# Nicholasli1995/EgoNet

Measured on AMD Instinct MI355X. Metric: crops/sec (256x256, heatmap+decode+lift), higher is better.
Workload: dtype f32; 1 GPU; configs[1]: batch=64 256x256 crops/GPU, HRNet-W48 heatmap head forward + soft decode + affine + FC lifter + pose solve; global_batch=64, weights=synthetic (egonet_amd.synth, seeded per key), parallelism=replicas x1, crops sharded by rank, no collective, ranks=1, backend=none, launch_lanes=1

## Files before the change

egonet_amd/_lib.py:

```python
import ctypes as C
import os

_HERE = os.path.dirname(os.path.abspath(__file__))
LIB_PATH = os.environ.get('EGONET_AMD_LIB') or os.path.join(_HERE, 'csrc', 'libegonet_hip.so')
HEADER_PATH = os.path.join(os.path.dirname(_HERE), 'include', 'egonet_hip.h')

ACT_NONE, ACT_RELU, ACT_SIGMOID, ACT_LEAKY = 0, 1, 2, 3


class Ref(C.Structure):
    _fields_ = [('slot', C.c_int32), ('off', C.c_int64)]


NULL_REF = Ref(-1, 0)

_p = C.c_void_p
_i = C.c_int
_d = C.c_double

SIGNATURES = {
    'egn_version': (_i, []),
    'egn_strerror': (C.c_char_p, [_i]),
    'egn_conv2d_f32': (_i, [_p] * 6 + [_i] * 14 + [_p]),
    'egn_conv_plan_query': (_i, [_i] * 13 + [C.POINTER(_i)]),
# ... 86 lines not shown
    'egn_optim_item_floats': (_i, []),
    'egn_optim_grouped_step_f32': (_i, [_i, _p, _p, _p, _p, _p, C.c_long, _p, _p, _i, _p, _p, C.c_long, _p, _p, _p]),
    'egn_grad_norm_ws_bytes': (C.c_long, []),
    'egn_grad_norm_clip_f32': (_i, [_p, C.c_long, C.c_float, _p, _p, _p]),
    'egn_program_create': (_p, [_i]),
    'egn_program_destroy': (None, [_p]),
    'egn_program_bind': (_i, [_p, _i, _p]),
    'egn_program_num_ops': (_i, [_p]),
    'egn_program_add_conv2d': (_i, [_p] + [Ref] * 6 + [_i] * 14),
    'egn_program_add_fuse': (_i, [_p, Ref, _i, _i, _i, _i, _i, _i, C.POINTER(Ref), C.POINTER(_i), _i]),
    'egn_program_add_nchw_to_nhwc': (_i, [_p, Ref, Ref, _i, _i, _i, _i, _i]),
    'egn_program_add_nhwc_to_nchw': (_i, [_p, Ref, Ref, _i, _i, _i, _i, _i]),
    'egn_program_add_pixel_shuffle': (_i, [_p, Ref, Ref, _i, _i, _i, _i, _i, _i]),
    'egn_program_add_pw_pair': (_i, [_p] + [Ref] * 8 + [_i, _i]),
    'egn_program_add_conv2d_pair': (_i, [_p] + ([Ref] * 6 + [_i] * 6) * 2 + [_i]),
    'egn_conv_pair_plan_query': (_i, [_i] * 13 + [C.POINTER(_i)]),
    'egn_conv3x3_h_applies': (_i, [_i] * 9),
    'egn_conv3x3_h_wpack_bytes': (C.c_long, [_i, _i]),
    'egn_conv3x3_h_f32': (_i, [_p] * 6 + [_i] * 6 + [_p]),
    'egn_program_add_conv3x3_h': (_i, [_p] + [Ref] * 6 + [_i] * 6),
    'egn_conv3x3s2_h_applies': (_i, [_i] * 8),
    'egn_conv3x3s2_h_f32': (_i, [_p] * 5 + [_i] * 6 + [_p]),
    'egn_program_add_conv3x3s2_h': (_i, [_p] + [Ref] * 5 + [_i] * 6),
    'egn_conv3x3_hx_applies': (_i, [_i] * 10),
    'egn_conv3x3_hx_wpack_bytes': (C.c_long, [_i, _i]),
    'egn_conv3x3_hx_f32': (_i, [_p] * 6 + [_i] * 7 + [_p]),
    'egn_program_add_conv3x3_hx': (_i, [_p] + [Ref] * 6 + [_i] * 7),
    'egn_pw_pair_f32': (_i, [_p] * 8 + [_i, _i, _p]),
    'egn_program_add_ramps': (_i, [_p, Ref, _i, _i, _i, _i, _i]),
    'egn_program_add_decode': (_i, [_p, Ref, _i, _i, _i, _i, _i, Ref, Ref, Ref]),
    'egn_program_fork': (_i, [_p]),
    'egn_program_join': (_i, [_p]),
    'egn_program_set_lane': (_i, [_p, _i]),
    'egn_program_tag': (_i, [_p, C.c_char_p, _d, _d]),
    'egn_program_run': (_i, [_p, _p]),
    'egn_program_run_timed': (_i, [_p, _p, C.POINTER(C.c_float), _i]),
    'egn_program_capture': (_i, [_p, _p]),
    'egn_program_replay': (_i, [_p, _p]),
    'egn_program_ticket_ops': (_i, [_p]),
    'egn_program_poke_ticket': (_i, [_p, _i, _i, C.c_uint]),
    'egn_gemm_supported': (_i, [_i] * 7),
    'egn_gemm_ws_bytes': (C.c_long, [_i] * 4),
    'egn_gemm_f32': (_i, [_i, _p, _p, _p, _p] + [_i] * 7 + [_p, C.c_long, _p]),
    'egn_gemm_stats_rows': (C.c_long, [_i]),
    'egn_gemm_ex_f32': (_i, [_i, _p, _p, _p, _p, _p, _p, C.c_long] + [_i] * 7 + [_p, C.c_long, _p]),
    'egn_launch_count': (C.c_long, []),
    'egn_direct_conv_count': (C.c_long, []),
    'egn_lifter_pairs_ws_bytes': (C.c_long, [_i, _i]),
    'egn_lifter_pairs_f64': (_i, [_p, _p, _i, _p, _i, _p, _i, _d, _d, _i, _i, _p, C.c_long, _p, _p, _p, _p]),
    'egn_col_mean_std_ws_bytes': (C.c_long, [_i]),
    'egn_col_mean_std_f32': (_i, [_p, C.c_long, _i, _p, C.c_long, _p, _p, _p]),
    'egn_normalize_rows_f32': (_i, [_p, C.c_long, _i, _p, _p, _p]),
    'egn_gather_rows_f32': (_i, [_p, C.c_long, _i, _p, _i, _p, _p]),
    'egn_pose2d_annot_ws_bytes': (C.c_long, [_i]),
    'egn_pose2d_annot_f64': (_i, [_p, _p, _p, _i, _p, _i, _d, _d, _i, _d, _i, _d, _p, C.c_long] + [_p] * 9),
    'egn_lifter_metrics_ws_bytes': (C.c_long, [C.c_long]),
    'egn_lifter_metrics_reset': (_i, [_p, _i, _p]),
    'egn_lifter_metrics_update_f32': (_i, [_p, _p, C.c_long, _i, _i, _p, _p, _i, _p, C.c_long, _p, _p, _p]),
    'egn_kpt_metrics_ws_bytes': (C.c_long, [_i, _i]),
    'egn_kpt_metrics_reset': (_i, [_p, _p]),
    'egn_kpt_metrics_update_f32': (_i, [_p, _p, _i, _i, _i, _i, _i, _p, _p, _p, _p, _i, _d, _d, _p, C.c_long, _p, _p, _p,
                                        _p, _p]),
    'egn_angle_metrics_ws_bytes': (C.c_long, [C.c_long]),
    'egn_angle_metrics_reset': (_i, [_p, _p]),
    'egn_angle_metrics_update_f32': (_i, [_p, C.c_long, _i, _p, _p, C.c_long, _p, _p]),
    'egn_pnp_refine_f64': (_i, [_p] * 5 + [_i, _i, _d] + [_p] * 6 + [_p]),
# ... 55 lines not shown
```

egonet_amd/csrc/program.hip:

```cpp
#include <stdlib.h>
#include <string.h>

#include <string>
#include <atomic>
#include <vector>

#include "egn_internal.h"

extern "C" int egn_conv_config_kind(int cfg);

extern "C" int egn_version(void) { return (1 << 16) | 0; }

extern "C" const char* egn_strerror(int code) {
  if (code == 0) return "ok";
  if (code == EGN_E_BADARG) return "egonet_hip: bad argument / unsupported shape";
  if (code == EGN_E_LDS) return "egonet_hip: tile does not fit in LDS";
  if (code == EGN_E_STATE) return "egonet_hip: program in wrong state";
  if (code > 0) return hipGetErrorString((hipError_t)code);
  return "egonet_hip: unknown error";
}

static int fill_conv_args(ConvArgs& a, const float* x, const float* wpack, const float* scale,
                          const float* shift, const float* res, float* y, int N, int H, int W, int Cin,
                          int cs_in, int Cout, int cs_out, int KH, int KW, int stride, int pad, int act,
// ... 102 lines not shown
  int rc = fill_conv_args(a, nullptr, nullptr, nullptr, nullptr, nullptr, nullptr, N, H, W, Cin, cs_in, Cout,
                          cs_out, KH, KW, stride, pad, 0, out_nchw);
  if (rc) return rc;
  size_t lds;
  rc = egn_conv_plan(a, cfg, lds);
  if (rc) return rc;
  int tm, tn;
  egn_conv_config_info(cfg, &tm, &tn);
  const ConvConfig* cf = egn_conv_config(cfg);
  out[0] = cfg; out[1] = cf->wm; out[2] = cf->wn; out[3] = cf->mt; out[4] = cf->nt;
  out[5] = a.TH; out[6] = a.TW; out[7] = a.TNB; out[8] = a.tps; out[9] = (int)lds;
  out[10] = a.tiles_x * a.tiles_y * ((a.N + a.TNB - 1) / a.TNB);
  out[11] = (a.CoutP + tn - 1) / tn;
  if (egn_conv_config_kind(cfg) == 1 && egn_wino_cot(Cout)) out[11] = Cout / egn_wino_cot(Cout);
  return 0;
}

enum OpKind { OP_CONV = 1, OP_FUSE = 2, OP_NCHW2NHWC = 3, OP_NHWC2NCHW = 4, OP_RAMPS = 5, OP_DECODE = 6,
              OP_FORK = 7, OP_JOIN = 8, OP_PIXSHUF = 9, OP_PWPAIR = 10, OP_CONVPAIR = 11, OP_CONVH = 12, OP_CONVH2 = 13,
              OP_CONVHX = 14 };
constexpr int kMaxLanes = 4;

struct Op {
  int kind;
  int lane = 0;
  ConvArgs conv;
  ConvArgs conv2;
  ConvHArgs convh;
  int cfg;
  egn_ref r[12];
  int i[12];
  std::string tag;
  double flops, bytes;
};

struct egn_program {
  std::vector<void*> slots;
  std::vector<Op> ops;
  std::vector<void*> owned;
  hipGraph_t graph = nullptr;
  hipGraphExec_t exec = nullptr;
  int cur_lane = 0;
  hipStream_t side[kMaxLanes] = {nullptr, nullptr, nullptr, nullptr};
  hipEvent_t ev_fork = nullptr;
  hipEvent_t ev_join[kMaxLanes] = {nullptr, nullptr, nullptr, nullptr};
  hipEvent_t ev_done = nullptr;
  hipStream_t last_stream = nullptr;
  bool ran = false;
  std::vector<unsigned*> tickets;
  std::vector<size_t> ticket_words;
  unsigned** err_ptrs = nullptr;
  unsigned* err_dev = nullptr;
  unsigned* err_host = nullptr;
  hipStream_t init_stream = nullptr;
};

__global__ void egn_ticket_errors_kernel(unsigned** bufs, int n, unsigned* any) {
  unsigned e = 0;
  for (int k = threadIdx.x; k < n; k += 64)
    if (bufs[k][0]) { e = 1u; bufs[k][0] = 0u; }
  if (e) *any = 1u;
}

static int issue_ticket_check(egn_program* p, hipStream_t s) {
  if (p->tickets.empty()) return 0;
  if (!p->err_ptrs) {
    EGN_CHECK_HIP(hipMalloc(&p->err_ptrs, p->tickets.size() * sizeof(unsigned*)));
    EGN_CHECK_HIP(hipMalloc(&p->err_dev, sizeof(unsigned)));
    EGN_CHECK_HIP(hipHostMalloc(&p->err_host, sizeof(unsigned), hipHostMallocDefault));
    *p->err_host = 0u;
    EGN_CHECK_HIP(hipMemcpy(p->err_ptrs, p->tickets.data(), p->tickets.size() * sizeof(unsigned*), hipMemcpyHostToDevice));
    EGN_CHECK_HIP(hipMemset(p->err_dev, 0, sizeof(unsigned)));
  }
  hipLaunchKernelGGL(egn_ticket_errors_kernel, dim3(1), dim3(64), 0, s, p->err_ptrs, (int)p->tickets.size(), p->err_dev);
  EGN_CHECK_HIP(hipGetLastError());
  EGN_CHECK_HIP(hipMemcpyAsync(p->err_host, p->err_dev, sizeof(unsigned), hipMemcpyDeviceToHost, s));
  return 0;
}
// ... 25 lines not shown
static inline void* resolve(const egn_program* p, const egn_ref& r) {
  if (r.slot < 0) return nullptr;
  return (char*)p->slots[r.slot] + r.off;
}
static inline bool ref_ok(const egn_program* p, const egn_ref& r) {
  return r.slot < (int)p->slots.size();
}

extern "C" egn_program* egn_program_create(int nslots) {
  if (nslots < 1 || nslots > 64) return nullptr;
  egn_program* p = new egn_program();
  p->slots.assign(nslots, nullptr);
  return p;
}

static void wait_for_last_run(egn_program* p) {
  if (p->ev_done && p->ran) hipEventSynchronize(p->ev_done);
}

extern "C" void egn_program_destroy(egn_program* p) {
  if (!p) return;
  wait_for_last_run(p);
  if (p->exec) hipGraphExecDestroy(p->exec);
  if (p->graph) hipGraphDestroy(p->graph);
  for (void* d : p->owned) hipFree(d);
  if (p->err_ptrs) hipFree(p->err_ptrs);
  if (p->err_dev) hipFree(p->err_dev);
  if (p->err_host) hipHostFree(p->err_host);
  if (p->init_stream) hipStreamDestroy(p->init_stream);
  for (int k = 1; k < kMaxLanes; ++k) {
    if (p->side[k]) hipStreamDestroy(p->side[k]);
    if (p->ev_join[k]) hipEventDestroy(p->ev_join[k]);
  }
  if (p->ev_fork) hipEventDestroy(p->ev_fork);
  if (p->ev_done) hipEventDestroy(p->ev_done);
  delete p;
}

extern "C" int egn_program_bind(egn_program* p, int slot, void* base) {
  if (!p || slot < 0 || slot >= (int)p->slots.size()) return EGN_E_BADARG;
  if (p->slots[slot] != base && p->exec) {
    wait_for_last_run(p);
    hipGraphExecDestroy(p->exec); p->exec = nullptr;
    hipGraphDestroy(p->graph); p->graph = nullptr;
  }
  p->slots[slot] = base;
  return 0;
}

extern "C" int egn_program_num_ops(const egn_program* p) { return p ? (int)p->ops.size() : 0; }

extern "C" int egn_program_add_conv2d(egn_program* p, egn_ref x, egn_ref wpack, egn_ref scale, egn_ref shift,
                                      egn_ref res, egn_ref y, int N, int H, int W, int Cin, int cs_in,
                                      int Cout, int cs_out, int KH, int KW, int stride, int pad, int act,
                                      int out_nchw, int cfg) {
  if (!p) return EGN_E_BADARG;
  Op op;
  op.kind = OP_CONV;
  op.flops = op.bytes = 0;
  int rc = fill_conv_args(op.conv, nullptr, nullptr, nullptr, nullptr, nullptr, nullptr, N, H, W, Cin, cs_in,
                          Cout, cs_out, KH, KW, stride, pad, act, out_nchw);
  if (rc) return rc;
  if (out_nchw && res.slot >= 0) return EGN_E_BADARG;
  size_t lds;
  rc = egn_conv_plan(op.conv, cfg, lds);
  if (rc) return rc;
// ... 208 lines not shown
  op.kind = OP_PWPAIR;
  op.r[0] = h; op.r[1] = res; op.r[2] = w3; op.r[3] = shift3; op.r[4] = w1; op.r[5] = shift1; op.r[6] = out; op.r[7] = hn;
  for (int k = 0; k < 8; ++k)
    if (!ref_ok(p, op.r[k])) return EGN_E_BADARG;
  op.i[0] = M; op.i[1] = relu1;
  op.flops = 2.0 * M * 64.0 * 256.0 * (w1.slot >= 0 ? 2.0 : 1.0);
  op.bytes = 4.0 * M * (64.0 + 256.0 * (res.slot >= 0 ? 2.0 : 1.0) + (w1.slot >= 0 ? 64.0 : 0.0));
  op.lane = p->cur_lane;
  p->ops.push_back(op);
  return 0;
}

extern "C" int egn_program_fork(egn_program* p) {
  if (!p) return EGN_E_BADARG;
  Op op;
  op.kind = OP_FORK;
  op.flops = op.bytes = 0;
  p->cur_lane = 0;
  p->ops.push_back(op);
  return 0;
}
extern "C" int egn_program_join(egn_program* p) {
  if (!p) return EGN_E_BADARG;
  Op op;
  op.kind = OP_JOIN;
  op.flops = op.bytes = 0;
  p->cur_lane = 0;
  p->ops.push_back(op);
  return 0;
}
extern "C" int egn_program_set_lane(egn_program* p, int lane) {
  if (!p || lane < 0 || lane >= kMaxLanes) return EGN_E_BADARG;
  p->cur_lane = lane;
  return 0;
}

extern "C" int egn_program_tag(egn_program* p, const char* tag, double flops, double bytes) {
  if (!p || p->ops.empty()) return EGN_E_STATE;
  Op& op = p->ops.back();
  op.tag = tag ? tag : "";
  if (flops > 0) op.flops = flops;
  op.bytes = bytes;
  return 0;
}

extern "C" int egn_program_op_info(const egn_program* p, int i, int* kind, double* flops, double* bytes,
                                   char* tag, int tag_len) {
  if (!p || i < 0 || i >= (int)p->ops.size()) return EGN_E_BADARG;
  const Op& op = p->ops[i];
  if (kind) *kind = op.kind;
  if (flops) *flops = op.flops;
  if (bytes) *bytes = op.bytes;
  if (tag && tag_len > 0) {
    strncpy(tag, op.tag.c_str(), tag_len - 1);
    tag[tag_len - 1] = 0;
  }
  return 0;
}

static std::atomic<long> g_launches{0};
static thread_local bool t_recording = false;
extern "C" long egn_launch_count(void) { return g_launches.load(std::memory_order_relaxed); }
void egn_count_launches(long n) { g_launches.fetch_add(n, std::memory_order_relaxed); }

static int launch_op(egn_program* p, Op& op, hipStream_t s) {
  if (!t_recording) g_launches.fetch_add(1, std::memory_order_relaxed);
// ... 35 lines not shown
      int shifts[4];
      for (int k = 0; k < op.i[5]; ++k) {
        terms[k] = (const float*)resolve(p, op.r[1 + k]);
        shifts[k] = op.i[6 + k];
      }
      return egn_fuse_sum_relu_f32((float*)resolve(p, op.r[0]), op.i[0], op.i[1], op.i[2], op.i[3], op.i[4],
                                   op.i[5], terms, shifts, op.i[10], s);
    }
    case OP_NCHW2NHWC:
      return egn_nchw_to_nhwc_f32((const float*)resolve(p, op.r[0]), (float*)resolve(p, op.r[1]), op.i[0],
                                  op.i[1], op.i[2], op.i[3], op.i[4], s);
    case OP_NHWC2NCHW:
      return egn_nhwc_to_nchw_f32((const float*)resolve(p, op.r[0]), (float*)resolve(p, op.r[1]), op.i[0],
                                  op.i[1], op.i[2], op.i[3], op.i[4], s);
    case OP_PIXSHUF:
      return egn_pixel_shuffle_nhwc_to_nchw_f32((const float*)resolve(p, op.r[0]), (float*)resolve(p, op.r[1]),
                                                op.i[0], op.i[1], op.i[2], op.i[3], op.i[4], op.i[5], s);
    case OP_RAMPS:
      return egn_fill_coord_ramps_f32((float*)resolve(p, op.r[0]), op.i[0], op.i[1], op.i[2], op.i[3],
                                      op.i[4], s);
    case OP_PWPAIR:
      return egn_pw_pair_f32((const float*)resolve(p, op.r[0]), (const float*)resolve(p, op.r[1]),
                             (const float*)resolve(p, op.r[2]), (const float*)resolve(p, op.r[3]),
                             (const float*)resolve(p, op.r[4]), (const float*)resolve(p, op.r[5]),
                             (float*)resolve(p, op.r[6]), (float*)resolve(p, op.r[7]), op.i[0], op.i[1], s);
    case OP_DECODE:
      return egn_decode_heatmaps_f32((const float*)resolve(p, op.r[0]), op.i[0], op.i[1], op.i[2], op.i[3],
                                     op.i[4], (float*)resolve(p, op.r[1]), (float*)resolve(p, op.r[2]),
                                     (int32_t*)resolve(p, op.r[3]), s);
  }
  return EGN_E_BADARG;
}

static int ensure_lanes(egn_program* p) {
  if (p->ev_fork) return 0;
  EGN_CHECK_HIP(hipEventCreateWithFlags(&p->ev_fork, hipEventDisableTiming));
  for (int k = 1; k < kMaxLanes; ++k) {
    EGN_CHECK_HIP(hipStreamCreateWithFlags(&p->side[k], hipStreamNonBlocking));
    EGN_CHECK_HIP(hipEventCreateWithFlags(&p->ev_join[k], hipEventDisableTiming));
  }
  return 0;
}

extern "C" int egn_program_run(egn_program* p, void* stream) {
  if (!p) return EGN_E_BADARG;
  hipStream_t main = (hipStream_t)stream;
  bool used[kMaxLanes] = {false, false, false, false};
  bool capturing = false;
  int rc_o = order_behind_last_run(p, main, &capturing);
  if (rc_o) return rc_o;
  if (!capturing) {
    rc_o = consume_ticket_error(p, main);
    if (rc_o) return rc_o;
  }
  for (Op& op : p->ops) {
    if (op.kind == OP_FORK) {
      int rc = ensure_lanes(p);
      if (rc) return rc;
      EGN_CHECK_HIP(hipEventRecord(p->ev_fork, main));
      for (int k = 1; k < kMaxLanes; ++k) used[k] = false;
      continue;
    }
    if (op.kind == OP_JOIN) {
      for (int k = 1; k < kMaxLanes; ++k)
        if (used[k]) {
          EGN_CHECK_HIP(hipEventRecord(p->ev_join[k], p->side[k]));
          EGN_CHECK_HIP(hipStreamWaitEvent(main, p->ev_join[k], 0));
          used[k] = false;
        }
      continue;
    }
    hipStream_t s = main;
    if (op.lane > 0 && p->ev_fork) {
      if (!used[op.lane]) {
        EGN_CHECK_HIP(hipStreamWaitEvent(p->side[op.lane], p->ev_fork, 0));
        used[op.lane] = true;
      }
      s = p->side[op.lane];
    }
    int rc = launch_op(p, op, s);
    if (rc) return rc;
  }
  if (!capturing || p->err_ptrs) {
    int rc = issue_ticket_check(p, main);
    if (rc) return rc;
  }
  return mark_run_issued(p, main, capturing);
}

extern "C" int egn_program_run_timed(egn_program* p, void* stream, float* ms, int n_ms) {
  if (!p || !ms || n_ms < (int)p->ops.size()) return EGN_E_BADARG;
  hipStream_t s = (hipStream_t)stream;
  const size_t n = p->ops.size();
  std::vector<hipEvent_t> ev(n + 1);
  for (auto& e : ev) EGN_CHECK_HIP(hipEventCreate(&e));
  bool capturing = false;
  int rc = order_behind_last_run(p, s, &capturing);
  if (!rc && capturing) rc = EGN_E_STATE;
  if (!rc) rc = consume_ticket_error(p, s);
  if (rc) { for (auto& e : ev) hipEventDestroy(e); return rc; }
  EGN_CHECK_HIP(hipEventRecord(ev[0], s));
  for (size_t i = 0; i < n && !rc; ++i) {
    if (p->ops[i].kind != OP_FORK && p->ops[i].kind != OP_JOIN) rc = launch_op(p, p->ops[i], s);
    if (!rc) rc = (int)hipEventRecord(ev[i + 1], s);
  }
  if (!rc) rc = issue_ticket_check(p, s);
  if (!rc) rc = mark_run_issued(p, s, false);
  if (!rc) rc = (int)hipStreamSynchronize(s);
  if (!rc)
    for (size_t i = 0; i < n; ++i) {
      float t = 0.f;
      hipEventElapsedTime(&t, ev[i], ev[i + 1]);
      ms[i] = t;
    }
  for (auto& e : ev) hipEventDestroy(e);
  return rc;
}

extern "C" int egn_program_ticket_ops(const egn_program* p) { return p ? (int)p->tickets.size() : 0; }
extern "C" int egn_program_poke_ticket(egn_program* p, int op, int word, unsigned value) {
  if (!p || op < 0 || op >= (int)p->tickets.size() || word < 0 || (size_t)word >= p->ticket_words[op]) return EGN_E_BADARG;
  wait_for_last_run(p);
  EGN_CHECK_HIP(hipMemcpy(p->tickets[op] + word, &value, sizeof(unsigned), hipMemcpyHostToDevice));
  return 0;
}

extern "C" int egn_program_capture(egn_program* p, void* stream) {
  if (!p) return EGN_E_BADARG;
  hipStream_t s = (hipStream_t)stream;
  if (p->exec) { wait_for_last_run(p); hipGraphExecDestroy(p->exec); p->exec = nullptr; }
  if (p->graph) { hipGraphDestroy(p->graph); p->graph = nullptr; }
  for (const Op& op : p->ops)
    if (op.kind == OP_FORK) {
      int rc0 = ensure_lanes(p);
      if (rc0) return rc0;
      break;
    }
  EGN_CHECK_HIP(hipStreamBeginCapture(s, hipStreamCaptureModeThreadLocal));
  t_recording = true;
  int rc = egn_program_run(p, stream);
  t_recording = false;
  hipGraph_t g = nullptr;
  hipError_t e = hipStreamEndCapture(s, &g);
  if (rc) { if (g) hipGraphDestroy(g); return rc; }
  if (e != hipSuccess) return (int)e;
  p->graph = g;
  EGN_CHECK_HIP(hipGraphInstantiate(&p->exec, p->graph, nullptr, nullptr, 0));
  return 0;
}

extern "C" int egn_program_replay(egn_program* p, void* stream) {
  if (!p || !p->exec) return EGN_E_STATE;
  long nk = 0;
  for (const Op& op : p->ops) nk += (op.kind != OP_FORK && op.kind != OP_JOIN);
  g_launches.fetch_add(nk, std::memory_order_relaxed);
  bool capturing = false;
  int rc = order_behind_last_run(p, (hipStream_t)stream, &capturing);
  if (rc) return rc;
  if (!capturing) {
    rc = consume_ticket_error(p, (hipStream_t)stream);
    if (rc) return rc;
  }
  EGN_CHECK_HIP(hipGraphLaunch(p->exec, (hipStream_t)stream));
  return mark_run_issued(p, (hipStream_t)stream, capturing);
}
```

egonet_amd/engine.py:

```python
import ctypes as C

import numpy as np
import torch
import torch.nn as nn

from . import _lib, tuner
from ._lib import Ref, NULL_REF, ACT_NONE, ACT_RELU, ACT_SIGMOID, ACT_LEAKY
from .filters import (CK, H_CK, H_KS, _round_up, pack_conv_weight, wino_cot, pack_wino_weight,
                      pack_wino43_weight, pack_wino4_weight, pack_conv_weight_f16, unpack_conv_weight_f16,
                      pack_conv_weight_f16x, unpack_conv_weight_f16x, pack_for_kind)

ACT_RES_AFTER = 0x10
BN_EPS_DEFAULT = 1e-5
SLOT_ARENA, SLOT_WEIGHTS, SLOT_USER0 = 0, 1, 2
PRECISIONS = ('f32', 'f16', 'f16s2')
F16S2_FP32_CLASSES = ((48, 48),)
ALL_PRECISIONS = PRECISIONS + ('f16x',)
_PRECISION_TEXT = "'f32', 'f16', 'f16s2' or 'f16x'"
F16X_FP32_CLASSES = ()


def _h_applies(n, h, w, cin, cs_in, cout, cs_out, has_res, act):
    return bool(_lib.lib().egn_conv3x3_h_applies(n, h, w, cin, cs_in, cout, cs_out, int(has_res), act))


def f16_eligible(conv, n, h, w):
    if not isinstance(conv, nn.Conv2d):
        return False
    if (tuple(conv.kernel_size), tuple(conv.stride), tuple(conv.padding), tuple(conv.dilation), conv.groups) != \
            ((3, 3), (1, 1), (1, 1), (1, 1), 1) or conv.bias is not None or conv.padding_mode != 'zeros':
        return False
    cin, cout = conv.in_channels, conv.out_channels
    return _h_applies(n, h, w, cin, cin, cout, cout, False, ACT_RELU)
# ... 89 lines not shown

def fold_pw(weight, bn):
    cout, cin = weight.shape[:2]
    scale, shift = fold_scale_shift(cout, None, bn)
    w = weight.detach().double().cpu().reshape(cout, cin) * scale[:cout].double()[:, None]
    return w.float().reshape(-1).contiguous(), shift[:cout].clone()


class Buf(object):
    __slots__ = ('n', 'h', 'w', 'c', 'cs', 'slot', 'off', 'nbytes', 'first', 'last', 'uses', 'name')

    def __init__(self, n, h, w, c, cs=None, slot=SLOT_ARENA, nbytes=None, name=''):
        self.n, self.h, self.w, self.c = n, h, w, c
        self.cs = _round_up(c, 4) if cs is None else cs
        self.slot = slot
        self.off = 0
        self.nbytes = nbytes if nbytes is not None else n * h * w * self.cs * 4
        self.first = self.last = -1
        self.uses = []
        self.name = name

    def ref(self):
        return Ref(self.slot, self.off)


class _Recorder(object):
    def __init__(self):
        self.ops = []
        self.blobs = []
        self.blob_off = 0
        self.bufs = []
        self.region = 0
        self.cur_lane = 0
        self.f16 = False
        self.f16s2 = False
        self.f16x = False

    def _push(self, kind, op):
        op['region'], op['lane'] = self.region, self.cur_lane
        self.ops.append((kind, op))

    def fork(self):
        self.region += 1
        self.cur_lane = 0
        self._push('fork', {})

    def lane(self, k):
        self.cur_lane = k % 4

    def join(self):
        self.cur_lane = 0
        self._push('join', {})
        self.region += 1

    def happens_before(self, u, d):
        (ru, lu), (rd, ld) = [(self.ops[i][1]['region'], self.ops[i][1]['lane']) for i in (u, d)]
        return ru < rd or (ru == rd and lu == ld and u < d)

    def new(self, n, h, w, c, name=''):
        b = Buf(n, h, w, c, name=name)
        self.bufs.append(b)
        return b

    def weight(self, t):
        off = self.blob_off
        self.blobs.append(t)
        self.blob_off += _round_up(t.numel() * 4, 256)
        return Ref(SLOT_WEIGHTS, off)

    def _touch(self, *bufs):
        i = len(self.ops)
        for b in bufs:
            if b is None:
                continue
            if b.first < 0:
                b.first = i
            b.last = i
            b.uses.append(i)

    def conv(self, x, weight, bias=None, bn=None, act=ACT_NONE, res=None, stride=1, pad=0,
             dst=None, out_nchw=False, cout_cs=None, tag=''):
        cout, cin, kh, kw = weight.shape
        assert cin == x.c, (cin, x.c, tag)
        ho = (x.h + 2 * pad - kh) // stride + 1
        wo = (x.w + 2 * pad - kw) // stride + 1
        dst_given = dst is not None
        if dst is None:
            dst = self.new(x.n, ho, wo, cout, name=tag)
            if cout_cs is not None:
                dst.cs = cout_cs
# ... 301 lines not shown
            x = op['x']
            _lib.check(L.egn_program_add_nhwc_to_nchw(h, x.ref(), op['y'], x.n, op['c'], x.h, x.w, x.cs))
            nbytes = 8.0 * x.n * x.h * x.w * op['c']
            klass = 'nhwc2nchw %d@%dx%d' % (op['c'], x.h, x.w)
        elif kind == 'pixshuf':
            x = op['x']
            _lib.check(L.egn_program_add_pixel_shuffle(h, x.ref(), op['y'], x.n, op['c'], x.h, x.w, x.cs, op['up']))
            nbytes = 8.0 * x.n * x.h * x.w * op['c'] * op['up'] ** 2
            klass = 'pixel_shuffle%d %d@%dx%d' % (op['up'], op['c'], x.h, x.w)
        elif kind == 'pwpair':
            hb, rb, ob, nb = op['h'], op['res'], op['out'], op['hn']
            none = NULL_REF
            _lib.check(L.egn_program_add_pw_pair(h, hb.ref(), rb.ref() if rb is not None else none, op['w3'], op['shift3'],
                                                 op['w1'] if nb is not None else none,
                                                 op['shift1'] if nb is not None else none, ob.ref(),
                                                 nb.ref() if nb is not None else none, op['m'], op['relu1']))
            flops = 2.0 * op['m'] * 64 * 256 * (2 if nb is not None else 1)
            nbytes = 4.0 * op['m'] * (64 + 256 * (2 if rb is not None else 1) + (64 if nb is not None else 0))
            klass = 'pwpair%d%d 64->256%s@%dx%d' % (int(rb is not None), op['relu1'], '->64' if nb is not None else '',
                                                    hb.h, hb.w)
        elif kind == 'ramps':
            y = op['y']
            _lib.check(L.egn_program_add_ramps(h, y.ref(), y.n, y.h, y.w, y.cs, op['c0']))
            nbytes = 8.0 * y.n * y.h * y.w
            klass = 'ramps'
        elif kind == 'decode':
            _lib.check(L.egn_program_add_decode(h, op['hm'], op['n'], op['k'], op['h'], op['w'],
                                                op['mode'], op['xy'], op['mx'], op['idx']))
            nbytes = 4.0 * op['n'] * op['k'] * op['h'] * op['w']
            klass = 'decode%d %dx%d' % (op['mode'], op['h'], op['w'])
        else:
            raise ValueError(kind)
        L.egn_program_tag(h, (op.get('tag') or klass).encode(), flops, nbytes)
        self.meta.append(dict(kind=kind, klass=klass, tag=op.get('tag', ''), flops=flops, bytes=nbytes,
                              cfg=op.get('cfg', 0) if kind == 'conv' else 0))

    def bind(self, slot, tensor):
        _lib.check(self.lib.egn_program_bind(self.handle, slot, _lib.ptr(tensor)))

    def run(self):
        _lib.check(self.lib.egn_program_run(self.handle, _lib.current_stream(self.device)), 'program_run')

    def run_timed(self):
        n = self.lib.egn_program_num_ops(self.handle)
        ms = (C.c_float * n)()
        _lib.check(self.lib.egn_program_run_timed(self.handle, _lib.current_stream(self.device), ms, n))
        return np.array(ms[:], dtype=np.float64)

    def capture(self):
        _lib.check(self.lib.egn_program_capture(self.handle, _lib.current_stream(self.device)))

    def replay(self):
        _lib.check(self.lib.egn_program_replay(self.handle, _lib.current_stream(self.device)))

    def __del__(self):
        try:
            if getattr(self, 'handle', None):
                self.lib.egn_program_destroy(self.handle)
                self.handle = None
        except Exception:
            pass


class _Stamp(object):

    def __init__(self, model):
# ... 10 lines not shown
            addr ^= t.data_ptr()
        return (ver, addr, len(self.tensors), getattr(self.model, '_egn_generation', 0),
                self.tensors[0].device if self.tensors else None)

    def changed(self):
        now = self._now()
        if now != self.last:
            self.tensors = None
            self.last = self._now()
            return True
        return False


def invalidate(model):
    model._egn_generation = getattr(model, '_egn_generation', 0) + 1
    model._engine = None


def _act_of(seq):
    return ACT_RELU if any(isinstance(m, nn.ReLU) for m in seq) else ACT_NONE


class HRNetEngine(object):

    def __init__(self, model):
        import os
        self.model = model
        self.programs = {}
        self._stamp = _Stamp(model)
        self.lanes = os.environ.get('EGONET_AMD_LANES', '1') != '0'
        self.graph_max_n = int(os.environ.get('EGONET_AMD_GRAPH_MAX_N', '0'))
        self.fuse_layer1 = os.environ.get('EGONET_AMD_PW_FUSE', '1') != '0'
        self.chain_regions = os.environ.get('EGONET_AMD_CHAIN', '1') != '0'
        self.last_f16_ops = []

    @property
    def precision(self):
        prec = getattr(self.model, 'precision', 'f32')
        if prec not in ALL_PRECISIONS:
            raise ValueError("precision must be %s, got %r" % (_PRECISION_TEXT, prec))
        return prec

    def _block(self, r, x, blk, tag):
        y = x
        for i in range(1, blk.depth + 1):
            conv = getattr(blk, 'conv%d' % i)
            bn = getattr(blk, 'bn%d' % i)
            k = conv.kernel_size[0]
            if i < blk.depth:
                y = r.conv(y, conv.weight, None, bn, ACT_RELU, None, conv.stride[0], conv.padding[0],
                           tag='%s.conv%d' % (tag, i))
            else:
                if blk.downsample is None:
                    res = x
                else:
                    pc, pb = blk.downsample[0], blk.downsample[1]
                    res = r.conv(x, pc.weight, None, pb, ACT_NONE, None, pc.stride[0], 0,
                                 tag=tag + '.downsample')
                y = r.conv(y, conv.weight, None, bn, ACT_RELU, res, conv.stride[0], conv.padding[0],
                           tag='%s.conv%d' % (tag, i))
        return y

    def _layer1(self, r, x, blocks):
        def plain():
            t = x
            for k, blk in enumerate(blocks):
# ... 46 lines not shown
            lowered = [any(r.takes_f16(x, conv.weight, conv.bias, ACT_RELU, None, conv.stride[0], conv.padding[0]) or
                           (getattr(r, 'f16x', False) and
                            r.takes_f16x(x, conv.weight, conv.bias, ACT_RELU, None, conv.stride[0], conv.padding[0]))
                           for blk in b for conv in (blk.conv1, blk.conv2) if getattr(blk, 'depth', 0) == 2)
                       for b, x in zip(mod.branches, xs)]

        def plain(branch, x):
            for blk in branch:
                if getattr(blk, 'depth', 0) != 2 or blk.downsample is not None:
                    return False
                for conv in (blk.conv1, blk.conv2):
                    if tuple(conv.weight.shape) != (x.c, x.c, 3, 3) or conv.stride[0] != 1 or conv.padding[0] != 1 \
                            or conv.bias is not None:
                        return False
            return x.cs == x.c and len(branch) > 0

        def key(x, has_res):
            return (x.n, x.h, x.w, x.c, x.c, x.c, x.c, 3, 3, 1, 1, has_res, False)
        nb = mod.num_branches
        for ia in reversed(range(nb)):
            for ib in reversed(range(nb)):
                if ia == ib or len(mod.branches[ia]) != len(mod.branches[ib]) or lowered[ia] or lowered[ib]:
                    continue
                if not (plain(mod.branches[ia], xs[ia]) and plain(mod.branches[ib], xs[ib])):
                    continue
                if all(tuner.pair_usable(key(xs[ia], res), key(xs[ib], res)) for res in (False, True)):
                    return ia, ib
        return None

    def _module(self, r, xs, mod, tag, region_open=False, keep_open=False, nxt=None):
        xs = list(xs)
        pair = self._pair_branches(r, xs, mod)
        lanes = self.lanes and mod.num_branches > 1
        if lanes and not region_open:
            r.fork()
        for b, branch in enumerate(mod.branches):
            if pair is not None and b == max(pair):
                continue
            if lanes:
                r.lane(b)
            if pair is not None and b == min(pair):
                ia, ib = pair
                for k, (ba, bb) in enumerate(zip(mod.branches[ia], mod.branches[ib])):
                    q = '%s.branches.%d+%d.%d' % (tag, ia, ib, k)
                    ha, hb = r.conv_pair(xs[ia], ba.conv1, ba.bn1, ACT_RELU, None,
                                         xs[ib], bb.conv1, bb.bn1, ACT_RELU, None, tag=q + '.conv1')
                    xs[ia], xs[ib] = r.conv_pair(ha, ba.conv2, ba.bn2, ACT_RELU, xs[ia],
                                                 hb, bb.conv2, bb.bn2, ACT_RELU, xs[ib], tag=q + '.conv2')
                continue
            for k, blk in enumerate(branch):
                xs[b] = self._block(r, xs[b], blk, '%s.branches.%d.%d' % (tag, b, k))
        if lanes:
            r.join()
        if mod.fuse_layers is None:
            return xs, False
        outs = []
        stay = lanes and keep_open and self.chain_regions and len(mod.fuse_layers) == mod.num_branches
        pair_next = self._pair_branches(r, xs, nxt) if stay else None
        if lanes:
            r.fork()
        for i, row in enumerate(mod.fuse_layers):
            if lanes:
                r.lane(min(pair_next) if pair_next is not None and i in pair_next else i)
            terms = []
            for j in range(mod.num_branches):
                q = '%s.fuse_layers.%d.%d' % (tag, i, j)
                if row[j] is None:
                    terms.append((xs[j], 0))
                elif j > i:
                    conv, bn = row[j][0], row[j][1]
                    t = r.conv(xs[j], conv.weight, None, bn, ACT_NONE, None, 1, 0, tag=q)
                    terms.append((t, j - i))
                else:
                    terms.append((self._unit_chain(r, xs[j], row[j], q), 0))
            outs.append(r.fuse(terms, True, tag='%s.fuse%d' % (tag, i)))
        if lanes and not stay:
            r.join()
        return outs, stay

    def _record(self, n, cin, h, w, decode_mode, r=None):
        m = self.model
        own = r is None
        if own:
            r = _Recorder()
            r.f16 = self.precision in ('f16', 'f16s2', 'f16x')
            r.f16s2 = self.precision in ('f16s2', 'f16x')
            r.f16x = self.precision == 'f16x'
        x = r.nchw_to_nhwc(Ref(SLOT_USER0, 0), n, cin, h, w, tag='input')
        t = r.conv(x, m.conv1.weight, None, m.bn1, ACT_RELU, None, 2, 1, tag='conv1')
        t = r.conv(t, m.conv2.weight, None, m.bn2, ACT_RELU, None, 2, 1, tag='conv2')
        t = self._layer1(r, t, m.layer1)
        ys = [t]
        for idx in (1, 2, 3):
            trans = getattr(m, 'transition%d' % idx)
            xs = []
            for i, tr in enumerate(trans):
                if tr is None:
                    xs.append(ys[i])
                elif isinstance(tr[0], nn.Conv2d):
                    xs.append(r.conv(ys[-1], tr[0].weight, None, tr[1], ACT_RELU, None, 1, 1,
                                     tag='transition%d.%d' % (idx, i)))
                else:
                    xs.append(self._unit_chain(r, ys[-1], tr, 'transition%d.%d' % (idx, i)))
            stage = getattr(m, 'stage%d' % (idx + 1))
            open_ = False
            for k, mod in enumerate(stage):
                nxt = stage[k + 1] if k + 1 < len(stage) else None
# ... 274 lines not shown
```

egonet_amd/tuner.py:

```python
import atexit
import ctypes as C
import functools
import json
import os

import torch

from . import _lib, filters

_HERE = os.path.dirname(os.path.abspath(__file__))
TABLE_PATH = os.path.join(_HERE, 'tuned', 'gfx950.json')
_table = None
_tuned_here = {}

DIRECT = frozenset((filters.DIRECT,))
ALL_KINDS = frozenset((filters.DIRECT, filters.WINO2, filters.WINO43, filters.WINO4))
TAPE_WINO, TAPE_F43 = frozenset((filters.DIRECT, filters.WINO2)), frozenset((filters.DIRECT, filters.WINO2, filters.WINO4))
F43_KINDS = frozenset((filters.WINO43, filters.WINO4))


def _load():
    global _table
    if _table is None:
        _table = {}
# ... 114 lines not shown
    fit = {int(k): v for k, v in entry.get('ms', {}).items() if ok(int(k))}
    return min(fit, key=fit.get) if fit else 0


def choose(device, key, kinds=DIRECT, ticket_cap=None, inplace_res=False):
    key, kinds = tuple(key), frozenset(kinds)
    mode = os.environ.get('EGONET_AMD_WINO', '')
    if os.environ.get('EGONET_AMD_F43', '1') == '0' or mode in ('0', '1'):
        kinds = kinds - F43_KINDS
    if mode == '0':
        kinds = DIRECT
    elif mode in ('1', '43', '43b', '43w'):
        first = {'43': (70, 80), '43b': (80, 70), '43w': (86, 80, 70)}.get(mode, ())
        ids = list(range(_lib.lib().egn_conv_num_configs(), 0, -1))
        for kind in sorted(kinds - DIRECT, reverse=True):
            for cfg in (list(first) if kind == filters.WINO4 else []) + ids:
                if kind_of(cfg) == kind and usable(key, cfg, kinds, ticket_cap, inplace_res):
                    return cfg
    name = shape_key(*key)
    only = os.environ.get('EGONET_AMD_F43_MATCH', '')
    if only and only not in name:
        kinds = kinds - F43_KINDS
    entry = _load().get(name)
    if entry is None:
        if os.environ.get('EGONET_AMD_AUTOTUNE', '1') == '0':
            return 0
        if name not in _tuned_here:
            cfg, times = tune(device, key)
            _tuned_here[name] = {'cfg': cfg, 'ms': {str(k): round(v, 5) for k, v in times.items()}}
        entry = _tuned_here[name]
    return _pick(entry, key, kinds, ticket_cap, inplace_res)


PAIRS_PATH = os.path.join(_HERE, 'tuned', 'gfx950_pairs.json')
PAIR_CFGS = (86, 82)
PAIR_DEFAULT = '0'
_pairs = None


def _load_pairs():
    global _pairs
    if _pairs is None:
        _pairs = {}
        try:
            with open(PAIRS_PATH) as f:
                _pairs = {k: v for k, v in json.load(f).items() if not k.startswith('_')}
        except (OSError, ValueError):
            _pairs = {}
    return _pairs


def pair_key(key_a, key_b):
    return shape_key(*key_a) + '+' + shape_key(*key_b)


def pair_plans(key_a, key_b, cus=256):
    if any(tuple(k[7:11]) != (3, 3, 1, 1) or k[3] != k[4] or k[5] != k[6] or k[12] for k in (key_a, key_b)):
        return None
    out = (C.c_int * 2)()
    rc = _lib.lib().egn_conv_pair_plan_query(*key_a[:4], key_a[5], *key_b[:4], key_b[5], cus, 0, 0, out)
    return (out[0], out[1]) if rc == 0 else None


def pair_usable(key_a, key_b):
    key_a, key_b = tuple(key_a), tuple(key_b)
    mode = os.environ.get('EGONET_AMD_PAIR', PAIR_DEFAULT)
# ... 90 lines not shown
```

include/egonet_hip.h:

```cpp
#ifndef EGONET_HIP_H
#define EGONET_HIP_H

#include <stdint.h>

#ifdef __cplusplus
extern "C" {
#endif

#define EGN_E_BADARG   (-1)
#define EGN_E_LDS      (-2)
#define EGN_E_STATE    (-3)

#define EGN_ACT_NONE    0
#define EGN_ACT_RELU    1
#define EGN_ACT_SIGMOID 2
#define EGN_ACT_LEAKY   3
#define EGN_ACT_MASK    0x0f
#define EGN_ACT_RES_AFTER 0x10

int egn_version(void);
const char* egn_strerror(int code);

int egn_conv2d_f32(const float* x, const float* wpack, const float* scale,
                   const float* shift, const float* res, float* y,
// ... 255 lines not shown
long egn_grad_norm_ws_bytes(void);
int egn_grad_norm_clip_f32(const float* g, long n, float max_norm, double* ws, float* clip, void* stream);

typedef struct egn_program egn_program;
typedef struct { int32_t slot; int64_t off; } egn_ref;

egn_program* egn_program_create(int nslots);
void egn_program_destroy(egn_program* p);
int egn_program_bind(egn_program* p, int slot, void* base);
int egn_program_num_ops(const egn_program* p);

int egn_program_add_conv2d(egn_program* p, egn_ref x, egn_ref wpack,
                           egn_ref scale, egn_ref shift, egn_ref res, egn_ref y,
                           int N, int H, int W, int Cin, int cs_in,
                           int Cout, int cs_out, int KH, int KW, int stride,
                           int pad, int act, int out_nchw, int cfg);
int egn_program_add_fuse(egn_program* p, egn_ref y, int N, int H, int W, int C,
                         int cs, int nterms, const egn_ref* terms,
                         const int* shifts, int relu);
int egn_program_add_nchw_to_nhwc(egn_program* p, egn_ref x, egn_ref y, int N,
                                 int C, int H, int W, int cs);
int egn_program_add_nhwc_to_nchw(egn_program* p, egn_ref x, egn_ref y, int N,
                                 int C, int H, int W, int cs);
int egn_program_add_pixel_shuffle(egn_program* p, egn_ref x, egn_ref y, int N,
                                  int C, int H, int W, int cs, int up);
int egn_program_add_ramps(egn_program* p, egn_ref y, int N, int H, int W,
                          int cs, int c0);
int egn_program_add_decode(egn_program* p, egn_ref hm, int N, int K, int H,
                           int W, int mode, egn_ref out_xy, egn_ref out_max,
                           egn_ref out_idx);
int egn_program_fork(egn_program* p);
int egn_program_join(egn_program* p);
int egn_program_set_lane(egn_program* p, int lane);
int egn_program_tag(egn_program* p, const char* tag, double flops, double bytes);

int egn_program_run(egn_program* p, void* stream);
int egn_program_run_timed(egn_program* p, void* stream, float* ms, int n_ms);
int egn_program_capture(egn_program* p, void* stream);
int egn_program_replay(egn_program* p, void* stream);
int egn_program_ticket_ops(const egn_program* p);
int egn_program_poke_ticket(egn_program* p, int op, int word, unsigned value);
int egn_program_add_pw_pair(egn_program* p, egn_ref h, egn_ref res, egn_ref w3, egn_ref shift3,
                            egn_ref w1, egn_ref shift1, egn_ref out, egn_ref hn, int M,
                            int relu1);
int egn_program_add_conv2d_pair(egn_program* p, egn_ref xa, egn_ref wa, egn_ref scale_a, egn_ref shift_a,
                                egn_ref res_a, egn_ref ya, int Na, int Ha, int Wa, int Cin_a, int Cout_a,
                                int act_a, egn_ref xb, egn_ref wb, egn_ref scale_b, egn_ref shift_b,
                                egn_ref res_b, egn_ref yb, int Nb, int Hb, int Wb, int Cin_b, int Cout_b,
                                int act_b, int grid_cap);
int egn_conv_pair_plan_query(int Na, int Ha, int Wa, int Cin_a, int Cout_a, int Nb, int Hb, int Wb,
                             int Cin_b, int Cout_b, int cus, int with_stats, int with_tickets, int* out);
int egn_conv3x3_h_applies(int N, int H, int W, int Cin, int cs_in, int Cout, int cs_out, int has_res, int act);
long egn_conv3x3_h_wpack_bytes(int Cin, int Cout);
int egn_conv3x3_h_f32(const float* x, const void* wpack_f16, const float* scale, const float* shift,
                      const float* res, float* y, int N, int H, int W, int Cin, int Cout, int act,
                      void* stream);
int egn_program_add_conv3x3_h(egn_program* p, egn_ref x, egn_ref wpack, egn_ref scale, egn_ref shift,
                              egn_ref res, egn_ref y, int N, int H, int W, int Cin, int Cout, int act);
int egn_conv3x3s2_h_applies(int N, int H, int W, int Cin, int cs_in, int Cout, int cs_out, int act);
int egn_conv3x3s2_h_f32(const float* x, const void* wpack_f16, const float* scale, const float* shift, float* y,
                        int N, int H, int W, int Cin, int Cout, int act, void* stream);
int egn_program_add_conv3x3s2_h(egn_program* p, egn_ref x, egn_ref wpack, egn_ref scale, egn_ref shift, egn_ref y,
                                int N, int H, int W, int Cin, int Cout, int act);
int egn_conv3x3_hx_applies(int N, int H, int W, int Cin, int cs_in, int Cout, int cs_out, int has_res, int act,
                           int stride);
long egn_conv3x3_hx_wpack_bytes(int Cin, int Cout);
// ... 81 lines not shown
```

Measured before the change: 5221 crops/s.

## Replace branch join/fork barrier with per-branch signal/wait dependencies

Adds per-op signal and wait events to the program runtime, with a Python signal/wait API. In HRNet multi-branch modules, the full join+fork between the branch convs and the fuse layers is dropped. Each fuse row instead waits only on the branches it consumes, visited in order of estimated finish time from tuned timings. The aim is to let fuse work start before the slowest branch finishes. Under graph capture, a wait on a signal recorded earlier in the same capture still falls back to a full lane join, which limits the overlap there.

```diff
diff --git a/egonet_amd/_lib.py b/egonet_amd/_lib.py
--- a/egonet_amd/_lib.py
+++ b/egonet_amd/_lib.py
@@ -142,6 +142,7 @@
     'egn_program_fork': (_i, [_p]),
     'egn_program_join': (_i, [_p]),
     'egn_program_set_lane': (_i, [_p, _i]),
+    'egn_program_set_deps': (_i, [_p, _i, C.POINTER(_i), _i]),
     'egn_program_tag': (_i, [_p, C.c_char_p, _d, _d]),
     'egn_program_run': (_i, [_p, _p]),
     'egn_program_run_timed': (_i, [_p, _p, C.POINTER(C.c_float), _i]),
diff --git a/egonet_amd/csrc/program.hip b/egonet_amd/csrc/program.hip
--- a/egonet_amd/csrc/program.hip
+++ b/egonet_amd/csrc/program.hip
@@ -158,6 +158,8 @@
   int i[12];
   std::string tag;
   double flops, bytes;
+  int signal = -1;
+  std::vector<int> waits;
 };
 
 struct egn_program {
@@ -170,6 +172,8 @@
   hipStream_t side[kMaxLanes] = {nullptr, nullptr, nullptr, nullptr};
   hipEvent_t ev_fork = nullptr;
   hipEvent_t ev_join[kMaxLanes] = {nullptr, nullptr, nullptr, nullptr};
+  int n_signals = 0;
+  std::vector<hipEvent_t> ev_sig;
   hipEvent_t ev_done = nullptr;
   hipStream_t last_stream = nullptr;
   bool ran = false;
@@ -261,6 +265,7 @@
     if (p->side[k]) hipStreamDestroy(p->side[k]);
     if (p->ev_join[k]) hipEventDestroy(p->ev_join[k]);
   }
+  for (hipEvent_t e : p->ev_sig) hipEventDestroy(e);
   if (p->ev_fork) hipEventDestroy(p->ev_fork);
   if (p->ev_done) hipEventDestroy(p->ev_done);
   delete p;
@@ -535,6 +540,22 @@
 extern "C" int egn_program_set_lane(egn_program* p, int lane) {
   if (!p || lane < 0 || lane >= kMaxLanes) return EGN_E_BADARG;
   p->cur_lane = lane;
+  return 0;
+}
+
+extern "C" int egn_program_set_deps(egn_program* p, int signal, const int* waits, int nwaits) {
+  if (!p || p->ops.empty()) return EGN_E_STATE;
+  if (nwaits < 0 || (nwaits > 0 && !waits)) return EGN_E_BADARG;
+  const int self = (int)p->ops.size() - 1;
+  Op& op = p->ops[self];
+  if (op.kind == OP_FORK || op.kind == OP_JOIN) return EGN_E_BADARG;
+  std::vector<int> evs;
+  for (int k = 0; k < nwaits; ++k) {
+    if (waits[k] < 0 || waits[k] >= self || p->ops[waits[k]].signal < 0) return EGN_E_BADARG;
+    evs.push_back(p->ops[waits[k]].signal);
+  }
+  op.waits = evs;
+  if (signal && op.signal < 0) op.signal = p->n_signals++;
   return 0;
 }
 
@@ -636,6 +657,15 @@
   return EGN_E_BADARG;
 }
 
+static int ensure_signals(egn_program* p) {
+  while ((int)p->ev_sig.size() < p->n_signals) {
+    hipEvent_t e = nullptr;
+    EGN_CHECK_HIP(hipEventCreateWithFlags(&e, hipEventDisableTiming));
+    p->ev_sig.push_back(e);
+  }
+  return 0;
+}
+
 static int ensure_lanes(egn_program* p) {
   if (p->ev_fork) return 0;
   EGN_CHECK_HIP(hipEventCreateWithFlags(&p->ev_fork, hipEventDisableTiming));
@@ -648,8 +678,10 @@
 
 extern "C" int egn_program_run(egn_program* p, void* stream) {
   if (!p) return EGN_E_BADARG;
+  { int rc_s = ensure_signals(p); if (rc_s) return rc_s; }
   hipStream_t main = (hipStream_t)stream;
   bool used[kMaxLanes] = {false, false, false, false};
+  std::vector<char> open_sig(p->n_signals, 0);
   bool capturing = false;
   int rc_o = order_behind_last_run(p, main, &capturing);
   if (rc_o) return rc_o;
@@ -672,7 +704,22 @@
           EGN_CHECK_HIP(hipStreamWaitEvent(main, p->ev_join[k], 0));
           used[k] = false;
         }
+      open_sig.assign(open_sig.size(), 0);
       continue;
+    }
+    if (capturing && p->ev_fork) {
+      bool need = false;
+      for (int w : op.waits) need = need || open_sig[w];
+      if (need) {
+        for (int k = 1; k < kMaxLanes; ++k)
+          if (used[k]) {
+            EGN_CHECK_HIP(hipEventRecord(p->ev_join[k], p->side[k]));
+            EGN_CHECK_HIP(hipStreamWaitEvent(main, p->ev_join[k], 0));
+            used[k] = false;
+          }
+        EGN_CHECK_HIP(hipEventRecord(p->ev_fork, main));
+        open_sig.assign(open_sig.size(), 0);
+      }
     }
     hipStream_t s = main;
     if (op.lane > 0 && p->ev_fork) {
@@ -682,8 +729,14 @@
       }
       s = p->side[op.lane];
     }
+    if (!capturing)
+      for (int w : op.waits) EGN_CHECK_HIP(hipStreamWaitEvent(s, p->ev_sig[w], 0));
     int rc = launch_op(p, op, s);
     if (rc) return rc;
+    if (op.signal >= 0) {
+      if (capturing) open_sig[op.signal] = 1;
+      else EGN_CHECK_HIP(hipEventRecord(p->ev_sig[op.signal], s));
+    }
   }
   if (!capturing || p->err_ptrs) {
     int rc = issue_ticket_check(p, main);
@@ -740,6 +793,7 @@
       if (rc0) return rc0;
       break;
     }
+  { int rc0 = ensure_signals(p); if (rc0) return rc0; }
   EGN_CHECK_HIP(hipStreamBeginCapture(s, hipStreamCaptureModeThreadLocal));
   t_recording = true;
   int rc = egn_program_run(p, stream);
diff --git a/egonet_amd/engine.py b/egonet_amd/engine.py
--- a/egonet_amd/engine.py
+++ b/egonet_amd/engine.py
@@ -1,4 +1,5 @@
 import ctypes as C
+import os
 
 import numpy as np
 import torch
@@ -154,13 +155,18 @@
         self.bufs = []
         self.region = 0
         self.cur_lane = 0
+        self._pending = {}
+        self._before = None
         self.f16 = False
         self.f16s2 = False
         self.f16x = False
 
     def _push(self, kind, op):
         op['region'], op['lane'] = self.region, self.cur_lane
+        if kind not in ('fork', 'join'):
+            op['waits'] = self._pending.pop(self.cur_lane, [])
         self.ops.append((kind, op))
+        self._before = None
 
     def fork(self):
         self.region += 1
@@ -171,13 +177,36 @@
         self.cur_lane = k % 4
 
     def join(self):
+        assert not self._pending, 'a wait with no op behind it on lanes %s' % sorted(self._pending)
         self.cur_lane = 0
         self._push('join', {})
         self.region += 1
 
+    def signal(self):
+        kind, op = self.ops[-1]
+        assert kind not in ('fork', 'join')
+        op['signal'] = True
+        return len(self.ops) - 1
+
+    def wait(self, token):
+        assert self.ops[token][1].get('signal'), token
+        self._pending.setdefault(self.cur_lane, []).append(token)
+
     def happens_before(self, u, d):
-        (ru, lu), (rd, ld) = [(self.ops[i][1]['region'], self.ops[i][1]['lane']) for i in (u, d)]
-        return ru < rd or (ru == rd and lu == ld and u < d)
+        if self.ops[u][1]['region'] < self.ops[d][1]['region']:
+            return True
+        if self._before is None:
+            before, last = [], {}
+            for i, (kind, op) in enumerate(self.ops):
+                at = (op['region'], op['lane'])
+                preds = ([last[at]] if at in last else []) + list(op.get('waits', ()))
+                m = 0
+                for p in preds:
+                    m |= before[p] | (1 << p)
+                before.append(m)
+                last[at] = i
+            self._before = before
+        return bool((self._before[d] >> u) & 1)
 
     def new(self, n, h, w, c, name=''):
         b = Buf(n, h, w, c, name=name)
@@ -545,6 +574,10 @@
         else:
             raise ValueError(kind)
         L.egn_program_tag(h, (op.get('tag') or klass).encode(), flops, nbytes)
+        if op.get('signal') or op.get('waits'):
+            waits = op.get('waits', [])
+            _lib.check(L.egn_program_set_deps(h, int(bool(op.get('signal'))), (C.c_int * len(waits))(*waits),
+                                              len(waits)), op.get('tag', ''))
         self.meta.append(dict(kind=kind, klass=klass, tag=op.get('tag', ''), flops=flops, bytes=nbytes,
                               cfg=op.get('cfg', 0) if kind == 'conv' else 0))
 
@@ -621,6 +654,8 @@
         self.graph_max_n = int(os.environ.get('EGONET_AMD_GRAPH_MAX_N', '0'))
         self.fuse_layer1 = os.environ.get('EGONET_AMD_PW_FUSE', '1') != '0'
         self.chain_regions = os.environ.get('EGONET_AMD_CHAIN', '1') != '0'
+        self.deps = os.environ.get('EGONET_AMD_DEPS', '1') != '0'
+        self.deps_min_n = int(os.environ.get('EGONET_AMD_DEPS_MIN_N', '16'))
         self.last_f16_ops = []
 
     @property
@@ -733,6 +768,9 @@
         xs = list(xs)
         pair = self._pair_branches(r, xs, mod)
         lanes = self.lanes and mod.num_branches > 1
+        deps = lanes and self.deps and hasattr(r, 'signal') and mod.fuse_layers is not None and \
+            xs[0].n >= self.deps_min_n and os.environ.get('EGONET_AMD_PAIR', tuner.PAIR_DEFAULT) == '0'
+        sig, eta = {}, {}
         if lanes and not region_open:
             r.fork()
         for b, branch in enumerate(mod.branches):
@@ -749,31 +787,39 @@
                     xs[ia], xs[ib] = r.conv_pair(ha, ba.conv2, ba.bn2, ACT_RELU, xs[ia],
                                                  hb, bb.conv2, bb.bn2, ACT_RELU, xs[ib], tag=q + '.conv2')
                 continue
+            first = len(r.ops) if deps else 0
             for k, blk in enumerate(branch):
                 xs[b] = self._block(r, xs[b], blk, '%s.branches.%d.%d' % (tag, b, k))
-        if lanes:
+            if deps:
+                assert len(r.ops) > first, 'branch %d of %s recorded no op to signal behind' % (b, tag)
+                sig[b] = r.signal()
+                eta[b] = sum(tuner.tabled_ms(Program._conv_key(op)) for kind, op in r.ops[first:] if kind == 'conv')
+        if lanes and not deps:
             r.join()
         if mod.fuse_layers is None:
             return xs, False
         outs = []
         stay = lanes and keep_open and self.chain_regions and len(mod.fuse_layers) == mod.num_branches
         pair_next = self._pair_branches(r, xs, nxt) if stay else None
-        if lanes:
+        if lanes and not deps:
             r.fork()
+        order = sorted(range(mod.num_branches), key=lambda j: (eta[j], j)) if deps else range(mod.num_branches)
         for i, row in enumerate(mod.fuse_layers):
             if lanes:
                 r.lane(min(pair_next) if pair_next is not None and i in pair_next else i)
-            terms = []
-            for j in range(mod.num_branches):
+            terms = [None] * mod.num_branches
+            for j in order:
                 q = '%s.fuse_layers.%d.%d' % (tag, i, j)
+                if deps and j != i:
+                    r.wait(sig[j])
                 if row[j] is None:
-                    terms.append((xs[j], 0))
+                    terms[j] = (xs[j], 0)
                 elif j > i:
                     conv, bn = row[j][0], row[j][1]
                     t = r.conv(xs[j], conv.weight, None, bn, ACT_NONE, None, 1, 0, tag=q)
-                    terms.append((t, j - i))
+                    terms[j] = (t, j - i)
                 else:
-                    terms.append((self._unit_chain(r, xs[j], row[j], q), 0))
+                    terms[j] = (self._unit_chain(r, xs[j], row[j], q), 0)
             outs.append(r.fuse(terms, True, tag='%s.fuse%d' % (tag, i)))
         if lanes and not stay:
             r.join()
diff --git a/egonet_amd/tuner.py b/egonet_amd/tuner.py
--- a/egonet_amd/tuner.py
+++ b/egonet_amd/tuner.py
@@ -170,6 +170,14 @@
     return _pick(entry, key, kinds, ticket_cap, inplace_res)
 
 
+def tabled_ms(key):
+    entry = _load().get(shape_key(*key))
+    if not entry:
+        return 0.0
+    ms = entry.get('ms', {})
+    return float(ms.get(str(entry.get('cfg')), min(ms.values()) if ms else 0.0))
+
+
 PAIRS_PATH = os.path.join(_HERE, 'tuned', 'gfx950_pairs.json')
 PAIR_CFGS = (86, 82)
 PAIR_DEFAULT = '0'
diff --git a/include/egonet_hip.h b/include/egonet_hip.h
--- a/include/egonet_hip.h
+++ b/include/egonet_hip.h
@@ -311,6 +311,7 @@
 int egn_program_fork(egn_program* p);
 int egn_program_join(egn_program* p);
 int egn_program_set_lane(egn_program* p, int lane);
+int egn_program_set_deps(egn_program* p, int signal, const int* waits, int nwaits);
 int egn_program_tag(egn_program* p, const char* tag, double flops, double bytes);
 
 int egn_program_run(egn_program* p, void* stream);
```

New measurement: 5273 crops/s, median of 6. +1.0%, better.
